# jac99/Egonn

Hardware: AMD Instinct MI355X
Metric: LiDAR scans/sec (descriptor extraction), 50k-pt clouds @ 0.1m voxel (higher is better)
Workload: dtype f32

## Files before the change

egonn_amd/_lib.py:

```python
from __future__ import annotations

import ctypes as C
import os
from typing import List, Optional, Sequence

import torch

_HERE = os.path.dirname(os.path.abspath(__file__))
LIB_PATH = os.path.join(_HERE, "lib", "libegonn_hip.so")

QUANT_CARTESIAN, QUANT_POLAR = 0, 1
FLAG_DISABLE_GLOBAL, FLAG_DISABLE_LOCAL, FLAG_IGNORE_KP_REGRESSOR, FLAG_BF16 = 1, 2, 4, 8
FLAG_POOL_SPOC, FLAG_POOL_MAC = 16, 32
MINKFPN_SPLIT_TOPDOWN = 1
MINKFPN_BLOCKS = {'BasicBlock': 0, 'ECABasicBlock': 1}
MINKFPN_POOLING = {None: 0, 'GeM': 1, 'MAC': 2, 'SPoC': 3}

_P = C.c_void_p
_SIGS = [
    ("egonn_ctx_create", C.c_int, [C.POINTER(_P), C.c_int, C.c_int]),
    ("egonn_ctx_destroy", None, [_P]),
    ("egonn_last_error", C.c_char_p, []),
    ("egonn_debug_set_naive_conv", C.c_int, [_P, C.c_int]),
    ("egonn_debug_set_ksplit", C.c_int, [_P, C.c_int, C.c_int, C.c_int, C.c_int, C.c_int]),
# ... 50 lines not shown
    ("egonn_minkfpn_finalize", C.c_int, [_P, C.c_int, C.POINTER(C.c_int), C.POINTER(C.c_int), C.c_int, C.c_int, C.c_int, C.c_int, _P]),
    ("egonn_minkfpn_out_level", C.c_int, [C.c_int, C.c_int, C.POINTER(C.c_int)]),
    ("egonn_minkfpn_forward", C.c_int, [_P, _P, C.c_int, _P, _P, _P]),
    ("egonn_topdown_step", C.c_int, [_P, C.c_int, _P, _P, _P, _P, C.c_int, C.c_int, _P, _P]),
    ("egonn_select_keypoints", C.c_int, [_P, _P, _P, _P, C.c_int, _P, _P, _P, _P, _P]),
    ("egonn_topk_rows", C.c_int, [_P, _P, C.c_int, C.c_int, _P, _P, _P]),
    ("egonn_triplet_loss_scratch_floats", C.c_int64, [C.c_int]),
    ("egonn_triplet_loss", C.c_int, [_P, C.c_int, C.c_int, _P, _P, C.c_float, _P, _P, _P, _P, _P]),
    ("egonn_nn_search", C.c_int, [_P, C.c_int64, _P, _P, C.c_int64, _P, _P, _P]),
    ("egonn_matrix_min", C.c_int, [_P, C.c_int64, C.c_int64, _P, _P, _P, _P, _P]),
    ("egonn_softmax_cross_entropy", C.c_int, [_P, C.c_int64, C.c_int64, _P, _P, _P, _P, _P]),
    ("egonn_local_loss_scratch_bytes", C.c_int64, [C.c_int, C.c_int64, C.c_int64, C.c_int]),
    ("egonn_local_loss", C.c_int, [C.c_int, C.c_int64, C.c_int64, C.c_int64, C.c_int64, C.c_int] + [_P] * 13 +
                                  [C.POINTER(C.c_float)] + [_P] * 9 + [C.c_int64, _P]),
    ("egonn_dense", C.c_int, [_P, C.c_int64, C.c_int, _P, C.c_int, _P, C.c_int, C.c_int, _P, _P]),
    ("egonn_dense_backward_weight", C.c_int, [_P, C.c_int, _P, C.c_int, C.c_int64, _P, _P, C.c_int64, _P]),
    ("egonn_conv_backward_weight", C.c_int, [_P, C.c_int, C.c_int, C.c_int, C.c_int, _P, C.c_int, _P, C.c_int, _P, _P,
                                             C.c_int64, _P]),
    ("egonn_col_stats", C.c_int, [C.c_int, _P, _P, _P, _P, C.c_int64, C.c_int, _P, _P, C.c_int64, _P]),
    ("egonn_bn_train_finalize", C.c_int, [_P, _P, C.c_double, C.c_int, _P, _P, C.c_float, C.c_float, _P, _P, _P, _P]),
    ("egonn_bn_backward_finalize", C.c_int, [_P, _P, C.c_double, C.c_int, _P, _P, _P, _P, _P]),
    ("egonn_affine_act", C.c_int, [_P, _P, _P, C.c_int64, C.c_int, C.c_int, _P, _P]),
    ("egonn_affine3", C.c_int, [_P, _P, _P, _P, _P, _P, C.c_int64, C.c_int, _P, _P]),
    ("egonn_relu_backward", C.c_int, [_P, _P, C.c_int64, C.c_int, _P, _P]),
    ("egonn_contrastive_loss_scratch_floats", C.c_int64, [C.c_int]),
    ("egonn_contrastive_loss", C.c_int, [_P, C.c_int, C.c_int, _P, _P, C.c_float, C.c_float, _P, _P, _P, _P, _P]),
    ("egonn_se_gate", C.c_int, [_P, _P, _P, _P, _P, C.c_int, C.c_int, C.c_int, _P, _P, _P]),
    ("egonn_se_gate_backward", C.c_int, [_P, _P, _P, _P, _P, _P, C.c_int, C.c_int, C.c_int, _P, _P, _P, _P, _P, _P]),
    ("egonn_eca_gate", C.c_int, [_P, _P, C.c_int, C.c_int, C.c_int, _P, _P]),
    ("egonn_eca_gate_backward", C.c_int, [_P, _P, _P, _P, C.c_int, C.c_int, C.c_int, _P, _P, _P]),
# ... 141 lines not shown
        raise ValueError(f"{name}: offsets must be a 1-D sequence of n_clouds + 1 entries, got shape {shape}")
    return shape[0] - 1


def concat_clouds(clouds, dev):
    ts = [torch.as_tensor(c) for c in clouds]
    for c in ts:
        check_cloud("cloud", c)
    off = [0]
    for c in ts:
        off.append(off[-1] + c.shape[0])
    pts = torch.cat([c.to(device=dev, dtype=torch.float32) for c in ts]) if ts else torch.zeros((0, 3), device=dev)
    return pts, torch.tensor(off, dtype=torch.int64, device=dev)


def debug_radix_sort(keys_in, vals_in, keys_out, vals_out, n: int, nbits: int, n_dev=None, seg_offsets=None, idx_bits: int = 0,
                     either_pair: bool = False, scratch_buf=None, scratch_bytes: Optional[int] = None) -> int:
    lib = load()
    B = 0 if seg_offsets is None else seg_offsets.numel() - 1
    need = lib.egonn_debug_radix_sort_scratch_bytes(int(n), B)
    if scratch_buf is None:
        scratch_buf = scratch(need, keys_in.device)
    pair = C.c_int32(-1)
    call(keys_in.device, lib.egonn_debug_radix_sort, keys_in.data_ptr(), vals_in.data_ptr(), keys_out.data_ptr(),
         vals_out.data_ptr(), int(n), int(nbits), _ptr(n_dev), _ptr(seg_offsets), B, int(idx_bits), int(bool(either_pair)),
         C.byref(pair), scratch_buf.data_ptr(), need if scratch_bytes is None else int(scratch_bytes))
    return pair.value


def require_gpu() -> torch.device:
# ... 561 lines not shown
```

egonn_amd/csrc/common.h:

```cpp
#pragma once
#include <hip/hip_runtime.h>
#include <atomic>
#include <stdint.h>
#include <stdio.h>
#include <string.h>
#include <string>
#include <vector>

#define EGONN_MAX_LEVELS 10
#define EGONN_NUM_LEVELS 8
#define EGONN_MAX_BATCH 4096

#define API extern "C" __attribute__((visibility("default")))

namespace egonn {

void set_error(const char* fmt, ...);
#define EGONN_OK 0
#define EGONN_ERR_INVALID 1
#define EGONN_ERR_HIP 2
#define EGONN_ERR_RANGE 3
#define EGONN_ERR_STATE 4
#define EGONN_ERR_CAPACITY 5
#define EGONN_ERR_FP16_RANGE 6
// ... 169 lines not shown
  hipEvent_t get();
};

struct Switches {
  bool debug_sync;
  bool no_presplit;
  bool no_fused_down;
  bool no_fused_lateral;
  bool no_gated_k2s2;
  bool no_fused_ghead;
  bool no_split_heads;
  bool no_tail_split;
  bool no_task_order;
  bool flat_sort, sort_pairs;
  bool no_search67;
  int split_max_level;
  int split_max_level_k8;
  int split_cfg;
  int rg_first_pass;
  const char* ksplit[5];
};
const Switches& switches();

struct KsRule {
  int8_t kparts[2][EGONN_NUM_LEVELS];
  int8_t kw[2][EGONN_NUM_LEVELS];
  int8_t col_parts[EGONN_NUM_LEVELS];
};

static constexpr int SCONV_RESIDENT_DEFAULT = 6;
// ... 76 lines not shown
```

egonn_amd/csrc/coords.hip:

```cpp
#include "common.h"

#include <algorithm>
#include <stdarg.h>

namespace egonn {

static thread_local char g_err[1024] = "";
void set_error(const char* fmt, ...) {
  va_list ap;
  va_start(ap, fmt);
  vsnprintf(g_err, sizeof(g_err), fmt, ap);
  va_end(ap);
}
const char* last_error() { return g_err; }

const Switches& switches() {
  static const Switches sw = [] {
    auto on = [](const char* name) { return getenv(name) != nullptr; };
    auto num = [](const char* name, int unset) { const char* e = getenv(name); return e ? atoi(e) : unset; };
    const char* ds = getenv("EGONN_DEBUG_SYNC");
    return Switches{.debug_sync = ds && ds[0] == '1', .no_presplit = on("EGONN_NO_PRESPLIT"), .no_fused_down = on("EGONN_NO_FUSED_DOWN"),
                    .no_fused_lateral = on("EGONN_NO_FUSED_LATERAL"), .no_gated_k2s2 = on("EGONN_NO_GATED_K2S2"),
                    .no_fused_ghead = on("EGONN_NO_FUSED_GHEAD"), .no_split_heads = on("EGONN_NO_SPLIT_HEADS"),
                    .no_tail_split = on("EGONN_NO_TAIL_SPLIT"), .no_task_order = on("EGONN_NO_TASK_ORDER"),
                    .flat_sort = on("EGONN_FLAT_SORT"), .sort_pairs = on("EGONN_SORT_PAIRS"), .no_search67 = on("EGONN_NO_SEARCH67"),
                    .split_max_level = num("EGONN_SPLIT_MAX_LEVEL", -1), .split_max_level_k8 = num("EGONN_SPLIT_MAX_LEVEL_K8", -1),
                    .split_cfg = num("EGONN_SPLIT_CFG", 0), .rg_first_pass = num("EGONN_RG_FIRST_PASS", 0),
                    .ksplit = {getenv("EGONN_KSPLIT"), getenv("EGONN_KSPLIT8"), getenv("EGONN_KSPLIT_KW"), getenv("EGONN_KSPLIT_KW8"),
                               getenv("EGONN_KSPLIT_PARTS")}};
  }();
  return sw;
}

hipEvent_t Profiler::get() {
  if (!pool.empty()) {
    hipEvent_t e = pool.back();
    pool.pop_back();
    return e;
  }
  hipEvent_t e = nullptr;
// ... 1037 lines not shown
```

egonn_amd/csrc/dense.hip:

```cpp
#include <algorithm>

#include "common.h"
#include "kernels.h"

namespace egonn {

typedef float f32x4 __attribute__((ext_vector_type(4)));

__device__ static inline float apply_act(float v, int act) {
  switch (act) {
    case ACT_RELU: return fmaxf(v, 0.f);
    case ACT_TANH: return tanhf(v);
    case ACT_SOFTPLUS: return v > 20.f ? v : log1pf(expf(v));
    case ACT_SIGMOID: return 1.f / (1.f + expf(-v));
    default: return v;
  }
}

__device__ static inline float bf2f(uint32_t h) { return __uint_as_float(h << 16); }
__device__ static inline uint32_t f2bf_rn(float a) {
  uint32_t u = __float_as_uint(a);
  u += 0x7FFFu + ((u >> 16) & 1u);
  return u >> 16;
}
// ... 338 lines not shown
          }
        }
        if (io & 2) {
          *reinterpret_cast<uint2*>(reinterpret_cast<uint16_t*>(out_v) + row * cout + c0) =
              make_uint2(f2bf_rn(v[0]) | (f2bf_rn(v[1]) << 16), f2bf_rn(v[2]) | (f2bf_rn(v[3]) << 16));
        } else {
          *reinterpret_cast<f32x4*>(reinterpret_cast<float*>(out_v) + row * cout + c0) = v;
        }
      }
    }
#pragma unroll
    for (int t = 0; t < KS; ++t) a[t] = an[t];
  }
}

__global__ void dense_any_kernel(const float* __restrict__ in, int64_t total, int cin, const float* __restrict__ W,
                                 int w_out_in, int cout, const float* __restrict__ bias, int act, float* __restrict__ out,
                                 const int32_t* __restrict__ n_dev) {
  const int64_t i = (int64_t)blockIdx.x * blockDim.x + threadIdx.x;
  if (n_dev) total = min((int64_t)*n_dev * cout, total);
  if (i >= total) return;
  const int64_t r = i / cout;
  const int co = (int)(i - r * cout);
  float s = bias ? bias[co] : 0.f;
  for (int ci = 0; ci < cin; ++ci) s = fmaf(in[r * cin + ci], w_out_in ? W[(int64_t)co * cin + ci] : W[(int64_t)ci * cout + co], s);
  out[i] = apply_act(s, act);
}

bool dense_gate_fusable(int64_t n, int cin, int cout) {
  const bool plan = cin == 32 || cin == 64 || cin == 96 || cin == 128 || cin == 192 || cin == 256;
  return plan && cout % 16 == 0 && n >= 8192 && (size_t)cin * cout * sizeof(float) <= 96 * 1024;
}

int dense_forward_ex(const void* in, int in_bf16, int64_t n, int cin, const float* W, int w_out_in, int cout,
                     const float* bias, const float* scale, const float* shift, int act, const void* residual, int res_bf16,
                     void* out, int out_bf16, hipStream_t stream, const int32_t* n_dev, const float* gate, const int32_t* boff,
                     int B) {
  if (n == 0) return EGONN_OK;
  EGONN_REQUIRE(!gate || (residual && boff && B >= 1 && dense_gate_fusable(n, cin, cout)), EGONN_ERR_INVALID,
                "dense: the fused gated residual needs the LDS-staged kernel (%lld rows, %d->%d)", (long long)n, cin, cout);
  const dim3 grid((unsigned)cdiv(n, 64), (unsigned)cdiv(cout, 64));
  const int io = (res_bf16 ? 1 : 0) | (out_bf16 ? 2 : 0);
  const size_t frag_bytes = (size_t)cin * cout * sizeof(float);
  const int ysplit = (int)cdiv((int64_t)frag_bytes, 96 * 1024);
  const int colblk = (int)(cdiv(cdiv(cout, ysplit), 16) * 16);
  if (cout % 16 == 0 && n >= (ysplit == 1 ? 8192 : 2048)) {
    const size_t blk_bytes = (size_t)cin * colblk * sizeof(float);
    const int ny = (int)cdiv(cout, colblk);
    const unsigned g1 = (unsigned)std::min<int64_t>(cdiv(cdiv(n, 16), 4), (blk_bytes > 72 * 1024 ? 256 : 512) / ny);
#define EGONN_DENSE_LDS_LAUNCH(WOI, CI, INB)                                                                           \
  {                                                                                                                   \
    static AttrOnce attr_done;                                                                                    \
    if (attr_done.need()) {                                                                                                 \
      HIP_CHECK(hipFuncSetAttribute(reinterpret_cast<const void*>(&dense_lds_kernel<WOI, CI, INB>),                   \
                                    hipFuncAttributeMaxDynamicSharedMemorySize, 160 * 1024));                         \
      attr_done.mark();                                                                                                \
    }                                                                                                                 \
// ... 981 lines not shown
  while (S < k) S <<= 1;
  const size_t lds = (size_t)(S + (k <= 512 ? k : 0)) * sizeof(unsigned long long);
  static AttrOnce attr_done;
  if (attr_done.need()) {
    HIP_CHECK(hipFuncSetAttribute(reinterpret_cast<const void*>(&select_topk_kernel), hipFuncAttributeMaxDynamicSharedMemorySize,
                                  128 * 1024));
    attr_done.mark(); 
  }
  hipLaunchKernelGGL(select_topk_kernel, dim3(B), dim3(TK_THREADS), lds, stream, sigma, boff_dev, k, S, kp, desc, dc, sel_rows,
                     sel_count, out_kp, out_desc);
  HIP_CHECK(hipGetLastError());
  return EGONN_OK;
}

}
```

egonn_amd/csrc/kernels.h:

```cpp
#pragma once
#include "common.h"

namespace egonn {

const char* last_error();

bool sconv_rg_supported(int cin, int cout);
int pack_rg_weights(const float* W, int K, int cin, int cout, int bf16, int flip, int transpose, void* out,
                    hipStream_t stream);
extern unsigned long long* g_sconv_trace;
struct PackedKernel {
  const void* rg32 = nullptr;
  const void* rg16 = nullptr;
  const void* split = nullptr;
};
struct ConvCall {
  int kind = 0, level = 0;
  const void* in = nullptr; void* out = nullptr;
  int cin = 0, cout = 0, bf16 = 0;
  const float *scale = nullptr, *shift = nullptr;
  int relu = 0;
  float* psum = nullptr;
  const PackedKernel* packed = nullptr;
  const float* W = nullptr; float* scratch = nullptr; size_t scratch_floats = 0;
// ... 44 lines not shown
int sconv_naive(const float* in, const int32_t* nbr, const float* W, const float* scale, const float* shift, int relu,
                float* out, int64_t n_out, int K, int cin, int cout, hipStream_t stream);
int conv0_lut_init(Ctx* ctx);
int conv0_k5_forward(Ctx* ctx, const float* feat, const float* W, int cout, const float* scale,
                     const float* shift, int relu, void* out, int out_bf16, hipStream_t stream, const void* wpk = nullptr);
int conv0_pack_unit(const float* W, void* wpk, hipStream_t stream);

enum Act { ACT_NONE = 0, ACT_RELU = 1, ACT_TANH = 2, ACT_SOFTPLUS = 3, ACT_SIGMOID = 4 };
int dense_forward(const float* in, int64_t n, int cin, const float* W, int w_out_in, int cout, const float* bias,
                  const float* scale, const float* shift, int act, const float* residual, float* out,
                  hipStream_t stream);
bool dense_gate_fusable(int64_t n, int cin, int cout);
int dense_forward_ex(const void* in, int in_bf16, int64_t n, int cin, const float* W, int w_out_in, int cout,
                     const float* bias, const float* scale, const float* shift, int act, const void* residual, int res_bf16,
                     void* out, int out_bf16, hipStream_t stream, const int32_t* n_dev = nullptr, const float* gate = nullptr,
                     const int32_t* boff = nullptr, int B = 0);
int bn_fold(const float* w, const float* b, const float* rm, const float* rv, float eps, int c, float* scale,
            float* shift, hipStream_t stream);
int gather_rows(const float* in, const int32_t* perm, int64_t n, int c, float* out, hipStream_t stream,
                const int32_t* n_dev = nullptr);
static constexpr int SEG_CHUNKS = 32;
int segment_partial_sums(const float* in, const int32_t* boff, int B, int c, int pow_mode, const float* p,
                         float* partial, hipStream_t stream);
int eca_apply(const float* x, const float* res, const float* partial, const int32_t* boff, int B, int64_t n, int c,
              const float* wconv, int ksize, float* out, hipStream_t stream);
int eca_gate_groups(const float* psum, const RowGroups& rg, const int32_t* boff, int B, int c, const float* wconv, int ksize,
                    float* gate, hipStream_t stream);
int eca_apply_gate(const void* x, const void* res, const float* gate, const int32_t* boff, int B, int64_t n, int c,
                   void* out, int bf16, hipStream_t stream);
int convert_bf16_to_f32(const void* in, int64_t n, float* out, hipStream_t stream);
int gem_finish(const float* partial, const int32_t* boff, int B, int c, const float* p, float* out,
// ... 34 lines not shown
```

egonn_amd/csrc/model.h:

```cpp
#pragma once
#include <map>
#include <string>
#include <vector>

#include "../../include/egonn_hip.h"
#include "common.h"
#include "kernels.h"

struct egonn_ctx : public egonn::Ctx {
  hipStream_t plan_stream = nullptr;

  void* level_feat[EGONN_NUM_LEVELS] = {};
  int level_ch[EGONN_NUM_LEVELS] = {};
  int level_bf16 = 0;
  bool from_points = false;
};

#define REQUIRE_PLAN(c)                                                                               \
  EGONN_REQUIRE((c) && (c)->plan.valid, EGONN_ERR_STATE, "no coordinate plan (call egonn_voxelize / " \
                                                         "egonn_coords_set first)")
#define REQUIRE_LEVEL(c, level)                                                                              \
  REQUIRE_PLAN(c);                                                                                           \
  HIP_CHECK(hipSetDevice((c)->device));                                                                      \
  EGONN_REQUIRE((level) >= 0 && (level) < EGONN_NUM_LEVELS, EGONN_ERR_INVALID, "level %d out of range", (level))
// ... 34 lines not shown
  float* folded = nullptr;
  size_t folded_cap = 0;
  const float* conv0 = nullptr;
  egonn::BnRef bn[8];
  const float* convs[8] = {};
  egonn::BlockRef blk[8];
  const float *g1x1[8] = {}, *gt[8] = {}, *l1x1[8] = {}, *lt[8] = {};
  const float* gem_p = nullptr;
  egonn::MlpRef gdec, ldec, kp, sg;
  float* packed = nullptr;
  size_t packed_cap = 0;
  void* conv0_unit = nullptr;
  void* lh_pack = nullptr;
  const float** lh_ptrs = nullptr;
  egonn::PackedKernel pk_convs[8], pk_c1[8], pk_c2[8], pk_gt[8], pk_lt[8];
  egonn::MinkFpnModel* fpn = nullptr;
};

namespace egonn {

int get_tensor(egonn_model* m, const std::string& key, std::initializer_list<int64_t> want, const float** out);
int get_bn(egonn_model* m, const std::string& prefix, int c, BnRef* bn, float** cursor);
int fold(const BnRef& bn, hipStream_t st);
int conv_layer(egonn_ctx* c, hipStream_t st, const ConvCall& cc, const char* what);
ConvCall conv_call(int kind, int level, const void* in, const PackedKernel& pk, int cin, int cout, int bf16, const BnRef* bn, int relu,
                   void* out);

bool topdown_split_supported(int C, int Cl);
int topdown_split_forward(Ctx* ctx, int level_out, const float* x_coarse, const void* sp_tconv, const float* x_lateral,
                          const void* sp_lateral, int C, int Cl, float* out, hipStream_t stream);
// ... 3 lines not shown
```

egonn_amd/csrc/model.hip:

```cpp
#include "model.h"

using namespace egonn;

namespace {

const int PLANES[7] = {32, 64, 64, 128, 128, 128, 128};
const int GLOBAL_CH = 128, GLOBAL_DIM = 256, LOCAL_CH = 64, LOCAL_DIM = 128;

}

API const char* egonn_last_error(void) { return last_error(); }

API int egonn_debug_set_naive_conv(egonn_ctx* c, int on) {
  EGONN_REQUIRE(c, EGONN_ERR_INVALID, "debug_set_naive_conv: null context");
  if (on >= 1000) { c->conv_variant = on; return EGONN_OK; }
  c->conv_variant = (on == 1) ? 3 : (on == 2 ? 1 : (on == 4 ? 2 : (on == 8 ? 4 : (on == 16 ? 5 : (on == 32 ? 6 : (on == 128 ? 9 : 0))))));
  return EGONN_OK;
}

API int egonn_debug_set_ksplit(egonn_ctx* c, int map_class, int level, int kparts, int kw, int col_parts) {
  EGONN_REQUIRE(c && (map_class == 0 || map_class == 1) && level >= 0 && level < EGONN_NUM_LEVELS, EGONN_ERR_INVALID,
                "debug_set_ksplit: bad argument");
  EGONN_REQUIRE(kparts <= 27 && kw <= 4 && col_parts <= 4, EGONN_ERR_INVALID, "debug_set_ksplit: kparts <= 27, kw <= 4, col_parts <= 4");
  if (kparts >= 0) c->ks_rule.kparts[map_class][level] = (int8_t)std::max(kparts, 1);
// ... 623 lines not shown
  EGONN_TRY(get_tensor(m, "local_head.tconv.4.kernel", {8, LOCAL_CH, LOCAL_CH}, &m->lt[4]));
  m->gem_p = nullptr;
  if (m->t.count("global_pooling.pooling.p")) EGONN_TRY(get_tensor(m, "global_pooling.pooling.p", {1}, &m->gem_p));
  EGONN_TRY(get_mlp(m, "global_descriptor_decoder", GLOBAL_CH, GLOBAL_DIM + (GLOBAL_CH - GLOBAL_DIM) / 2, GLOBAL_DIM, &m->gdec));
  EGONN_TRY(get_mlp(m, "local_descriptor_decoder", LOCAL_CH, LOCAL_DIM + (LOCAL_CH - LOCAL_DIM) / 2, LOCAL_DIM, &m->ldec));
  EGONN_TRY(get_mlp(m, "local_keypoint_regressor", LOCAL_CH, LOCAL_CH / 2, 3, &m->kp));
  EGONN_TRY(get_mlp(m, "local_sigma_regressor", LOCAL_CH, LOCAL_CH / 2, 1, &m->sg));

  {
    size_t need_p = 0;
    for (int i = 1; i <= 7; ++i) {
      const BlockRef& b = m->blk[i];
      need_p += (size_t)8 * b.cin * b.cin + (size_t)27 * b.cin * b.cout + (size_t)27 * b.cout * b.cout;
    }
    need_p += (size_t)2 * 8 * GLOBAL_CH * GLOBAL_CH + (size_t)8 * LOCAL_CH * LOCAL_CH;
    if (m->packed_cap < need_p) {
      if (m->packed) HIP_CHECK(hipFree(m->packed));
      HIP_CHECK(hipMalloc(reinterpret_cast<void**>(&m->packed), (3 * need_p + 512) * sizeof(float)));
      m->packed_cap = need_p;
    }
    float* pc = m->packed;
    uint16_t* qc = reinterpret_cast<uint16_t*>(m->packed + need_p);
    uint16_t* sc = reinterpret_cast<uint16_t*>(m->packed + need_p + need_p / 2 + 16);
    auto pack2 = [&](const float* w, int K, int ci, int co, PackedKernel* dst) -> int {
      EGONN_TRY(pack_rg_weights(w, K, ci, co, 0, 0, 0, pc, st));
      EGONN_TRY(pack_rg_weights(w, K, ci, co, 1, 0, 0, qc, st));
      *dst = PackedKernel{pc, qc, nullptr};
      if (sconv_split_supported(ci, co)) {
        EGONN_TRY(pack_split_weights(w, K, ci, co, 0, 0, sc, st));
        dst->split = sc;
        sc += split_weights_bytes(K, ci, co) / 2;
      }
      pc += (size_t)K * ci * co;
      qc += (size_t)K * ci * co;
      return EGONN_OK;
    };
    for (int i = 1; i <= 7; ++i) {
      const BlockRef& b = m->blk[i];
      EGONN_TRY(pack2(m->convs[i], 8, b.cin, b.cin, &m->pk_convs[i]));
      EGONN_TRY(pack2(b.conv1, 27, b.cin, b.cout, &m->pk_c1[i]));
      EGONN_TRY(pack2(b.conv2, 27, b.cout, b.cout, &m->pk_c2[i]));
    }
    EGONN_TRY(pack2(m->gt[6], 8, GLOBAL_CH, GLOBAL_CH, &m->pk_gt[6]));
    EGONN_TRY(pack2(m->gt[7], 8, GLOBAL_CH, GLOBAL_CH, &m->pk_gt[7]));
    EGONN_TRY(pack2(m->lt[4], 8, LOCAL_CH, LOCAL_CH, &m->pk_lt[4]));
  }
  if (!m->conv0_unit) HIP_CHECK(hipMalloc(&m->conv0_unit, 2 * 4 * 3 * 64 * 16));
  EGONN_TRY(conv0_pack_unit(m->conv0, m->conv0_unit, st));
  if (m->ldec.cin == 64 && m->ldec.mid == 96 && m->ldec.cout == 128 && m->kp.mid == 32 && m->sg.mid == 32 && m->kp.cin == 64 &&
      m->sg.cin == 64) {
    if (!m->lh_pack) HIP_CHECK(hipMalloc(&m->lh_pack, local_heads_pack_bytes()));
    if (!m->lh_ptrs) HIP_CHECK(hipMalloc(reinterpret_cast<void**>(&m->lh_ptrs), 6 * sizeof(float*)));
    const float* hp[6] = {m->ldec.w0, m->ldec.w1, m->kp.w0, m->kp.w1, m->sg.w0, m->sg.w1};
    HIP_CHECK(hipMemcpyAsync(m->lh_ptrs, hp, sizeof(hp), hipMemcpyHostToDevice, st));
    HIP_CHECK(hipStreamSynchronize(st));
    EGONN_TRY(local_heads_pack(m->lh_ptrs, m->lh_pack, st));
  }
  EGONN_TRY(fold(m->bn[0], st));
  for (int i = 1; i <= 7; ++i) {
    EGONN_TRY(fold(m->bn[i], st));
// ... 99 lines not shown
  }
  FALLOC(x0, n0 * 32);
  {
    ProfScope ps(c, st, "conv0_k5_kernel/L0", PK_CONV0, 0, 125, 1, 32, (int)es);
    EGONN_TRY(conv0_k5_forward(c, f0, m->conv0, 32, m->bn[0].scale, m->bn[0].shift, 1, x0, bf16, st, m->conv0_unit));
  }
  DBG_SYNC("conv0");
  const void* x[8] = {x0};
  c->level_feat[0] = x0;
  c->level_ch[0] = 32;
  c->level_bf16 = bf16;
  auto local_head = [&](hipStream_t st) -> int {
    const int64_t n3 = P.cap[3], n4 = P.cap[4];
    FALLOC(l4, n4 * LOCAL_CH);
    EGONN_TRY(dense_forward_ex(x[4], bf16, n4, 128, m->l1x1[4], 0, LOCAL_CH, nullptr, nullptr, nullptr, ACT_NONE, nullptr, 0, l4,
                               bf16, st, cnt + 4));
    FALLOC(u3, n3 * LOCAL_CH);
    EGONN_TRY(conv_layer(c, st, conv_call(2, 3, l4, m->pk_lt[4], LOCAL_CH, LOCAL_CH, bf16, nullptr, 0, u3), "tconv"));
    EGONN_REQUIRE(m->ldec.cin == 64 && m->ldec.mid == 96 && m->ldec.cout == 128 && m->kp.mid == 32 && m->sg.mid == 32,
                  EGONN_ERR_STATE, "local heads: unexpected layer sizes");
    const float* hw[12] = {m->ldec.w0, m->ldec.b0, m->ldec.w1, m->ldec.b1, m->kp.w0, m->kp.b0, m->kp.w1, m->kp.b1,
                           m->sg.w0, m->sg.b0, m->sg.w1, m->sg.b1};
    const void* lh_pack = (!switches().no_split_heads && sconv_split_arithmetic(c)) ? m->lh_pack : nullptr;
    if (!switches().no_fused_lateral && LOCAL_CH == 64) {
      EGONN_TRY(local_heads_forward(reinterpret_cast<const float*>(x[3]), n3, cnt + 3, hw, P.lv[3].keys, 3, P.coord_bits, quant_mode,
                                    step, (flags & EGONN_FLAG_IGNORE_KP_REGRESSOR) ? 1 : 0, out_desc, out_kp, out_sigma, st,
                                    m->l1x1[3], reinterpret_cast<const float*>(u3), bf16, lh_pack, c->dev_fp16_flag));
      return EGONN_OK;
    }
    WALLOC(l3, n3 * LOCAL_CH);
    EGONN_TRY(dense_forward_ex(x[3], bf16, n3, 64, m->l1x1[3], 0, LOCAL_CH, nullptr, nullptr, nullptr, ACT_NONE, u3, bf16, l3, 0, st, cnt + 3));
    EGONN_TRY(local_heads_forward(l3, n3, cnt + 3, hw, P.lv[3].keys, 3, P.coord_bits, quant_mode, step,
                                  (flags & EGONN_FLAG_IGNORE_KP_REGRESSOR) ? 1 : 0, out_desc, out_kp, out_sigma, st, nullptr, nullptr, 0,
                                  lh_pack, c->dev_fp16_flag));
    return EGONN_OK;
  };
  const float *gated_t2 = nullptr, *gated_res = nullptr, *gated_gate = nullptr;
  for (int i = 1; i <= 7; ++i) {
    const BlockRef& b = m->blk[i];
    const Level& L = P.lv[i];
    const int64_t n = P.cap[i];
    FALLOC(y, n * b.cin);
    {
      ConvCall cc = conv_call(1, i, x[i - 1], m->pk_convs[i], b.cin, b.cin, bf16, &m->bn[i], 1, y);
      if (gated_t2 && i == 2) {
        cc.in = gated_t2;
// ... 25 lines not shown
    DBG_SYNC("L%d eca gate", i);
    const void* res = y;
    if (i == 1 && !switches().no_gated_k2s2 && !c->keep_level_features && !bf16 && !b.down && c->conv_variant == 0 && b.cout == 32 &&
        m->blk[2].cin == 32 && sconv_route(c, 1, 2, 32, 32, 0) == ROUTE_SPLIT) {
      gated_t2 = reinterpret_cast<const float*>(t2);
      gated_res = reinterpret_cast<const float*>(y);
      gated_gate = gate;
      x[i] = nullptr;
      c->level_feat[i] = nullptr;
      c->level_ch[i] = b.cout;
      continue;
    }
    FALLOC(xo, n * b.cout);
    if (b.down && !switches().no_fused_down && dense_gate_fusable(n, b.cin, b.cout)) {
      EGONN_TRY(dense_forward_ex(y, bf16, n, b.cin, b.down, 0, b.cout, nullptr, b.dn.scale, b.dn.shift, ACT_NONE, t2, bf16, xo,
                                 bf16, st, cnt + i, gate, L.boff, B));
    } else {
      if (b.down) {
        FALLOC(rd, n * b.cout);
        EGONN_TRY(dense_forward_ex(y, bf16, n, b.cin, b.down, 0, b.cout, nullptr, b.dn.scale, b.dn.shift, ACT_NONE, nullptr, 0, rd,
                                   bf16, st, cnt + i));
        res = rd;
      }
      EGONN_TRY(eca_apply_gate(t2, res, gate, L.boff, B, n, b.cout, xo, bf16, st));
    }
    DBG_SYNC("L%d eca apply", i);
    x[i] = xo;
    c->level_feat[i] = xo;
    c->level_ch[i] = b.cout;
  }
  if (do_local) EGONN_TRY(local_head(st));
  DBG_SYNC("local head");

  void* g5_fused = nullptr;
  if (do_global && !switches().no_fused_ghead && !bf16 && c->conv_variant == 0 && P.cap[5] < 8192 && P.cap[6] < 8192 && P.cap[7] < 8192) {
    WALLOC(l7, P.cap[7] * GLOBAL_CH);
// ... 146 lines not shown
```

include/egonn_hip.h:

```cpp
#ifndef EGONN_HIP_H
#define EGONN_HIP_H

#include <stdint.h>

#ifdef __cplusplus
extern "C" {
#endif

typedef struct egonn_ctx egonn_ctx;
typedef struct egonn_model egonn_model;

enum { EGONN_QUANT_CARTESIAN = 0, EGONN_QUANT_POLAR = 1 };
enum { EGONN_STATUS_OK = 0, EGONN_STATUS_INVALID = 1, EGONN_STATUS_HIP = 2, EGONN_STATUS_RANGE = 3, EGONN_STATUS_STATE = 4,
       EGONN_STATUS_CAPACITY = 5,
       EGONN_STATUS_FP16_RANGE = 6 };
enum { EGONN_FLAG_DISABLE_GLOBAL = 1, EGONN_FLAG_DISABLE_LOCAL = 2, EGONN_FLAG_IGNORE_KP_REGRESSOR = 4,
       EGONN_FLAG_BF16 = 8,
       EGONN_FLAG_POOL_SPOC = 16, EGONN_FLAG_POOL_MAC = 32 };

int egonn_ctx_create(egonn_ctx** ctx, int device, int coord_bits);
void egonn_ctx_destroy(egonn_ctx* ctx);
const char* egonn_last_error(void);
int egonn_debug_set_naive_conv(egonn_ctx* ctx, int on);
int egonn_debug_set_ksplit(egonn_ctx* ctx, int map_class, int level, int kparts, int kw, int col_parts);
// ... 120 lines not shown
       EGONN_LL_CHAMFER_WEIGHTED = 4, EGONN_LL_MEAN_SIGMA = 5, EGONN_LL_LOSS_CHAMFER = 6, EGONN_LL_LOSS_P2P = 7,
       EGONN_LL_KEYPOINT_LOSS = 8, EGONN_LL_CORRESPONDENCE_LOSS = 9, EGONN_LL_MATCHING_KEYPOINTS = 10,
       EGONN_LL_MATCHING_DESCRIPTORS = 11, EGONN_LL_POS_SIMILARITY = 12, EGONN_LL_NEG_SIMILARITY = 13  };
int64_t egonn_local_loss_scratch_bytes(int pairs, int64_t n_kp1, int64_t n_kp2, int dim);
int egonn_local_loss(int pairs, int64_t n_cloud1, int64_t n_cloud2, int64_t n_kp1, int64_t n_kp2, int dim,
                     const float* clouds1, const int32_t* cloud_off1, const float* clouds2, const int32_t* cloud_off2,
                     const float* kp1, const float* sigma1, const float* desc1, const int32_t* kp_off1,
                     const float* kp2, const float* sigma2, const float* desc2, const int32_t* kp_off2,
                     const float* transforms, const float* params, float* out_pair, float* out_batch,
                     float* g_kp1, float* g_sigma1, float* g_desc1, float* g_kp2, float* g_sigma2, float* g_desc2,
                     void* scratch, int64_t scratch_bytes, void* stream);

enum { EGONN_ACT_NONE = 0, EGONN_ACT_RELU = 1, EGONN_ACT_TANH = 2, EGONN_ACT_SOFTPLUS = 3, EGONN_ACT_SIGMOID = 4 };
int egonn_dense(const float* x, int64_t n, int cin, const float* weight, int weight_out_in, const float* bias, int cout,
                int act, float* out, void* stream);
int egonn_dense_backward_weight(const float* a, int ca, const float* b, int cb, int64_t n, float* out, float* scratch,
                                int64_t scratch_floats, void* stream);
int egonn_conv_backward_weight(egonn_ctx* ctx, int level_in, int level_out, int kernel_size, int transposed,
                               const float* in, int cin, const float* grad_out, int cout, float* grad_kernel,
                               float* scratch, int64_t scratch_floats, void* stream);
int egonn_col_stats(int mode, const float* a, const float* b, const float* mask, const float* mean, int64_t n, int c,
                    double* out, float* scratch, int64_t scratch_floats, void* stream);
int egonn_bn_train_finalize(const double* sums, const float* shift_point, double count, int c, const float* weight,
                            const float* bias, float eps, float momentum, float* running_mean, float* running_var,
                            float* out_mean_invstd_scale_shift, void* stream);
int egonn_bn_backward_finalize(const double* local_sums, const double* global_sums, double count, int c, const float* weight,
                               const float* mean, const float* invstd, float* out_abc_dgamma_dbeta, void* stream);
int egonn_affine_act(const float* x, const float* scale, const float* shift, int64_t n, int c, int relu, float* out,
                     void* stream);
int egonn_affine3(const float* g, const float* mask, const float* x, const float* A, const float* B, const float* C,
// ... 157 lines not shown
```

Measured before the change: 22450.

## Add streaming MFMA dense kernel with prepacked weight fragments for 1x1 layers

Adds a dense (1x1 conv) kernel specialised by template on channel count. Each wave handles 16 rows, loads the whole weight matrix into LDS as MFMA-ready fragments, and fuses bias, scale/shift, activation, residual and gated residual into the epilogue. The weights for the downsample and lateral 1x1 layers are packed into fragment order once at model finalize, so the kernel skips the per-launch reordering. This aims to cut per-row overhead and register tiling waste for large point counts. It adds template instantiations, more LDS per block, and a new default path for n>=8192 that can be turned off with EGONN_NO_DENSE_STREAM.

```diff
diff --git a/egonn_amd/_lib.py b/egonn_amd/_lib.py
--- a/egonn_amd/_lib.py
+++ b/egonn_amd/_lib.py
@@ -4,6 +4,7 @@
 import os
 from typing import List, Optional, Sequence
 
+import numpy as np
 import torch
 
 _HERE = os.path.dirname(os.path.abspath(__file__))
@@ -88,6 +89,10 @@
     ("egonn_local_loss", C.c_int, [C.c_int, C.c_int64, C.c_int64, C.c_int64, C.c_int64, C.c_int] + [_P] * 13 +
                                   [C.POINTER(C.c_float)] + [_P] * 9 + [C.c_int64, _P]),
     ("egonn_dense", C.c_int, [_P, C.c_int64, C.c_int, _P, C.c_int, _P, C.c_int, C.c_int, _P, _P]),
+    ("egonn_dense_pack_fragments", C.c_int, [_P, C.c_int, C.c_int, C.c_int, _P, _P]),
+    ("egonn_dense_pack_fragments_host", C.c_int, [_P, C.c_int, C.c_int, C.c_int, _P]),
+    ("egonn_debug_dense", C.c_int, [_P, C.c_int, C.c_int64, _P, C.c_int, C.c_int, _P, C.c_int, _P, _P, _P, _P, C.c_int, _P, C.c_int,
+                                    _P, _P, C.c_int, _P, C.c_int, C.c_int, _P]),
     ("egonn_dense_backward_weight", C.c_int, [_P, C.c_int, _P, C.c_int, C.c_int64, _P, _P, C.c_int64, _P]),
     ("egonn_conv_backward_weight", C.c_int, [_P, C.c_int, C.c_int, C.c_int, C.c_int, _P, C.c_int, _P, C.c_int, _P, _P,
                                              C.c_int64, _P]),
@@ -259,6 +264,33 @@
     return pts, torch.tensor(off, dtype=torch.int64, device=dev)
 
 
+def dense_pack_fragments(weight, out_in: bool):
+    lib = load()
+    co, ci = (weight.shape if out_in else weight.shape[::-1])
+    if isinstance(weight, np.ndarray):
+        w = np.ascontiguousarray(weight, dtype=np.float32)
+        out = np.empty(ci * co, dtype=np.float32)
+        check(lib.egonn_dense_pack_fragments_host(w.ctypes.data, int(bool(out_in)), int(ci), int(co), out.ctypes.data))
+        return out
+    w = weight.contiguous()
+    out = torch.empty(ci * co, dtype=torch.float32, device=w.device)
+    call(w.device, lib.egonn_dense_pack_fragments, w.data_ptr(), int(bool(out_in)), int(ci), int(co), out.data_ptr())
+    return out
+
+
+def debug_dense(x, weight, out_in: bool, out, form: int, n_dev=None, packed=None, bias=None, scale=None, shift=None, act: int = 0,
+                residual=None, gate=None, boff=None):
+    lib = load()
+    cap, cin = x.shape
+    cout = out.shape[1]
+    B = 0 if boff is None else boff.numel() - 1
+    bf = lambda t: int(t is not None and t.dtype == torch.bfloat16)
+    call(x.device, lib.egonn_debug_dense, x.data_ptr(), bf(x), int(cap), _ptr(n_dev), int(cin), int(cout), weight.data_ptr(),
+         int(bool(out_in)), _ptr(packed), _ptr(bias), _ptr(scale), _ptr(shift), int(act), _ptr(residual), bf(residual), _ptr(gate),
+         _ptr(boff), B, out.data_ptr(), bf(out), int(form))
+    return out
+
+
 def debug_radix_sort(keys_in, vals_in, keys_out, vals_out, n: int, nbits: int, n_dev=None, seg_offsets=None, idx_bits: int = 0,
                      either_pair: bool = False, scratch_buf=None, scratch_bytes: Optional[int] = None) -> int:
     lib = load()
diff --git a/egonn_amd/csrc/common.h b/egonn_amd/csrc/common.h
--- a/egonn_amd/csrc/common.h
+++ b/egonn_amd/csrc/common.h
@@ -207,6 +207,7 @@
   bool no_task_order;
   bool flat_sort, sort_pairs;
   bool no_search67;
+  bool no_dense_stream;
   int split_max_level;
   int split_max_level_k8;
   int split_cfg;
diff --git a/egonn_amd/csrc/coords.hip b/egonn_amd/csrc/coords.hip
--- a/egonn_amd/csrc/coords.hip
+++ b/egonn_amd/csrc/coords.hip
@@ -24,6 +24,7 @@
                     .no_fused_ghead = on("EGONN_NO_FUSED_GHEAD"), .no_split_heads = on("EGONN_NO_SPLIT_HEADS"),
                     .no_tail_split = on("EGONN_NO_TAIL_SPLIT"), .no_task_order = on("EGONN_NO_TASK_ORDER"),
                     .flat_sort = on("EGONN_FLAT_SORT"), .sort_pairs = on("EGONN_SORT_PAIRS"), .no_search67 = on("EGONN_NO_SEARCH67"),
+                    .no_dense_stream = on("EGONN_NO_DENSE_STREAM"),
                     .split_max_level = num("EGONN_SPLIT_MAX_LEVEL", -1), .split_max_level_k8 = num("EGONN_SPLIT_MAX_LEVEL_K8", -1),
                     .split_cfg = num("EGONN_SPLIT_CFG", 0), .rg_first_pass = num("EGONN_RG_FIRST_PASS", 0),
                     .ksplit = {getenv("EGONN_KSPLIT"), getenv("EGONN_KSPLIT8"), getenv("EGONN_KSPLIT_KW"), getenv("EGONN_KSPLIT_KW8"),
diff --git a/egonn_amd/csrc/dense.hip b/egonn_amd/csrc/dense.hip
--- a/egonn_amd/csrc/dense.hip
+++ b/egonn_amd/csrc/dense.hip
@@ -376,6 +376,163 @@
   }
 }
 
+__host__ __device__ static inline int64_t dense_frag_src(int64_t j, int w_out_in, int cin, int cout) {
+  const int u = (int)(j & 3), ln = (int)((j >> 2) & 63), ft = (int)(j >> 8), ks = cin / 16;
+  const int nt = ft / ks, t = ft - nt * ks;
+  const int ci = 16 * t + 4 * (ln >> 4) + u, col = 16 * nt + (ln & 15);
+  return w_out_in ? (int64_t)col * cin + ci : (int64_t)ci * cout + col;
+}
+__global__ void dense_pack_kernel(const float* __restrict__ W, int w_out_in, int cin, int cout, float* __restrict__ out) {
+  const int64_t j = (int64_t)blockIdx.x * blockDim.x + threadIdx.x;
+  if (j < (int64_t)cin * cout) out[j] = W[dense_frag_src(j, w_out_in, cin, cout)];
+}
+int dense_pack_frags(const float* W, int w_out_in, int cin, int cout, float* out, hipStream_t stream) {
+  EGONN_REQUIRE(W && out && cin >= 16 && cin % 16 == 0 && cout >= 16 && cout % 16 == 0, EGONN_ERR_INVALID,
+                "dense pack: %d->%d (multiples of 16 expected)", cin, cout);
+  hipLaunchKernelGGL(dense_pack_kernel, dim3((unsigned)cdiv((int64_t)cin * cout, 256)), dim3(256), 0, stream, W, w_out_in ? 1 : 0, cin,
+                     cout, out);
+  HIP_CHECK(hipGetLastError());
+  return EGONN_OK;
+}
+
+template <int CIN, int COUT, bool IN_BF16, bool ACT_ANY>
+__global__ __launch_bounds__(256, 4) void dense_stream_kernel(const void* __restrict__ in_v, int64_t n, const float* __restrict__ W,
+                                                           int w_out_in, const float* __restrict__ wfrag,
+                                                           const float* __restrict__ bias, const float* __restrict__ scale,
+                                                           const float* __restrict__ shift, int act,
+                                                           const void* __restrict__ residual_v, void* __restrict__ out_v, int io,
+                                                           const int32_t* __restrict__ n_dev, const float* __restrict__ gate,
+                                                           const int32_t* __restrict__ boff, int B) {
+  extern __shared__ __attribute__((aligned(16))) f32x4 ds_frags[];
+  constexpr int KS = CIN / 16, NT = COUT / 16, NFRAG = NT * KS * 64, PER = NFRAG / 256;
+  static_assert(NFRAG % 256 == 0, "whole fragments per thread");
+  float* const s_vec = reinterpret_cast<float*>(ds_frags + NFRAG);
+  int32_t* const s_boff = reinterpret_cast<int32_t*>(s_vec + 3 * COUT);
+  if (n_dev) n = min((int64_t)*n_dev, n);
+  if (!gate) B = 0;
+  const int tid = threadIdx.x, lane = tid & 63, wave = tid >> 6;
+  const int l15 = lane & 15, g4 = lane >> 4;
+  f32x4 st[PER];
+  {
+    const f32x4* src = reinterpret_cast<const f32x4*>(wfrag ? wfrag : W);
+#pragma unroll
+    for (int u = 0; u < PER; ++u) st[u] = src[tid + u * 256];
+  }
+  const int vi = min(tid, COUT - 1);
+  float vb = (bias ? bias : W)[vi], vs = (scale ? scale : W)[vi], vh = (scale ? shift : W)[vi];
+  const int32_t vo = (gate ? boff : reinterpret_cast<const int32_t*>(W))[gate ? min(tid, B) : 0];
+  const int64_t row = ((int64_t)blockIdx.x * 4 + wave) * 16 + l15;
+  const bool ok = row < n;
+  const int64_t rowc = min(row, max(n, (int64_t)1) - 1);
+  f32x4 a[KS], r[NT];
+#pragma unroll
+  for (int t = 0; t < KS; ++t) {
+    if constexpr (IN_BF16) {
+      const uint2 h = *reinterpret_cast<const uint2*>(reinterpret_cast<const uint16_t*>(in_v) + rowc * CIN + 16 * t + 4 * g4);
+      a[t] = (f32x4){__uint_as_float(h.x), __uint_as_float(h.y), 0.f, 0.f};
+    } else {
+      a[t] = *reinterpret_cast<const f32x4*>(reinterpret_cast<const float*>(in_v) + rowc * CIN + 16 * t + 4 * g4);
+    }
+  }
+  {
+    const void* rp = residual_v ? residual_v : static_cast<const void*>(W);
+    const int64_t r0 = (residual_v ? rowc * COUT : 0) + 4 * g4;
+    if (io & 1) {
+#pragma unroll
+      for (int nt = 0; nt < NT; ++nt) {
+        const uint2 h = *reinterpret_cast<const uint2*>(reinterpret_cast<const uint16_t*>(rp) + r0 + 16 * nt);
+        r[nt] = (f32x4){__uint_as_float(h.x), __uint_as_float(h.y), 0.f, 0.f};
+      }
+    } else {
+#pragma unroll
+      for (int nt = 0; nt < NT; ++nt) r[nt] = *reinterpret_cast<const f32x4*>(reinterpret_cast<const float*>(rp) + r0 + 16 * nt);
+    }
+  }
+#pragma unroll
+  for (int u = 0; u < PER; ++u) ds_frags[tid + u * 256] = st[u];
+  if (!wfrag) {
+#pragma unroll 1
+    for (int i = tid; i < NFRAG; i += 256) {
+      f32x4 v;
+#pragma unroll
+      for (int k = 0; k < 4; ++k) v[k] = W[dense_frag_src((int64_t)i * 4 + k, w_out_in, CIN, COUT)];
+      ds_frags[i] = v;
+    }
+  }
+  if (tid < COUT) {
+    s_vec[tid] = bias ? vb : 0.f;
+    s_vec[COUT + tid] = scale ? vs : 1.f;
+    s_vec[2 * COUT + tid] = scale ? vh : 0.f;
+  }
+  if (tid <= B) s_boff[tid] = vo;
+  for (int i = tid + 256; i <= B; i += 256) s_boff[i] = boff[i];
+  __syncthreads();
+  if (((int64_t)blockIdx.x * 4 + wave) * 16 >= n) return;
+  f32x4 gq[NT];
+  {
+    int lo = 0, hi = gate ? B : 0;
+    while (hi - lo > 1) {
+      const int mid = (lo + hi) >> 1;
+      if (s_boff[mid] <= (int32_t)row) lo = mid; else hi = mid;
+    }
+    const float* gp = (gate ? gate : W) + ((gate && ok) ? (int64_t)lo * COUT : 0) + 4 * g4;
+#pragma unroll
+    for (int nt = 0; nt < NT; ++nt) gq[nt] = *reinterpret_cast<const f32x4*>(gp + 16 * nt);
+  }
+  __builtin_amdgcn_sched_barrier(0);
+  if constexpr (IN_BF16) {
+#pragma unroll
+    for (int t = 0; t < KS; ++t) {
+      const uint32_t hx = __float_as_uint(a[t][0]), hy = __float_as_uint(a[t][1]);
+      a[t] = (f32x4){bf2f(hx & 0xFFFFu), bf2f(hx >> 16), bf2f(hy & 0xFFFFu), bf2f(hy >> 16)};
+    }
+  }
+#pragma unroll
+  for (int nt = 0; nt < NT; ++nt) {
+    f32x4 acc = {0.f, 0.f, 0.f, 0.f};
+    const f32x4* fr = ds_frags + nt * KS * 64 + lane;
+#pragma unroll
+    for (int t = 0; t < KS; ++t) {
+      const f32x4 wf = fr[t * 64];
+#pragma unroll
+      for (int u = 0; u < 4; ++u) acc = __builtin_amdgcn_mfma_f32_16x16x4f32(wf[u], a[t][u], acc, 0, 0, 0);
+    }
+    if (ok) {
+      const int c0 = 16 * nt + 4 * g4;
+      f32x4 v = acc + *reinterpret_cast<const f32x4*>(s_vec + c0);
+      v = v * *reinterpret_cast<const f32x4*>(s_vec + COUT + c0) + *reinterpret_cast<const f32x4*>(s_vec + 2 * COUT + c0);
+#pragma unroll
+      for (int u = 0; u < 4; ++u) v[u] = ACT_ANY ? apply_act(v[u], act) : (act == ACT_RELU ? fmaxf(v[u], 0.f) : v[u]);
+      if (residual_v) {
+        f32x4 rr = r[nt];
+        if (io & 1) {
+          const uint32_t hx = __float_as_uint(rr[0]), hy = __float_as_uint(rr[1]);
+          rr = (f32x4){bf2f(hx & 0xFFFFu), bf2f(hx >> 16), bf2f(hy & 0xFFFFu), bf2f(hy >> 16)};
+        }
+        if (gate) {
+#pragma unroll
+          for (int u = 0; u < 4; ++u) {
+            const float d = (io & 2) ? bf2f(f2bf_rn(v[u])) : v[u];
+            v[u] = fmaxf(rr[u] * gq[nt][u] + d, 0.f);
+          }
+        } else {
+          v += rr;
+        }
+      }
+      if (io & 2) {
+        *reinterpret_cast<uint2*>(reinterpret_cast<uint16_t*>(out_v) + row * COUT + c0) =
+            make_uint2(f2bf_rn(v[0]) | (f2bf_rn(v[1]) << 16), f2bf_rn(v[2]) | (f2bf_rn(v[3]) << 16));
+      } else {
+        *reinterpret_cast<f32x4*>(reinterpret_cast<float*>(out_v) + row * COUT + c0) = v;
+      }
+    }
+    __builtin_amdgcn_sched_barrier(0);
+  }
+}
+static bool dense_stream_shape(int64_t n, int cin, int cout) {
+  return n >= 8192 && (cin == 32 || cin == 64 || cin == 128) && (cout == 64 || cout == 128) && (size_t)cin * cout * sizeof(float) <= 32 * 1024;
+}
+
 __global__ void dense_any_kernel(const float* __restrict__ in, int64_t total, int cin, const float* __restrict__ W,
                                  int w_out_in, int cout, const float* __restrict__ bias, int act, float* __restrict__ out,
                                  const int32_t* __restrict__ n_dev) {
@@ -397,12 +554,39 @@
 int dense_forward_ex(const void* in, int in_bf16, int64_t n, int cin, const float* W, int w_out_in, int cout,
                      const float* bias, const float* scale, const float* shift, int act, const void* residual, int res_bf16,
                      void* out, int out_bf16, hipStream_t stream, const int32_t* n_dev, const float* gate, const int32_t* boff,
-                     int B) {
+                     int B, const float* wfrag, int form) {
   if (n == 0) return EGONN_OK;
   EGONN_REQUIRE(!gate || (residual && boff && B >= 1 && dense_gate_fusable(n, cin, cout)), EGONN_ERR_INVALID,
                 "dense: the fused gated residual needs the LDS-staged kernel (%lld rows, %d->%d)", (long long)n, cin, cout);
+  EGONN_REQUIRE(form != 1 || dense_stream_shape(n, cin, cout), EGONN_ERR_INVALID, "dense: no streaming form for %lld rows, %d->%d",
+                (long long)n, cin, cout);
   const dim3 grid((unsigned)cdiv(n, 64), (unsigned)cdiv(cout, 64));
   const int io = (res_bf16 ? 1 : 0) | (out_bf16 ? 2 : 0);
+  if (form == 1 || (form < 0 && !switches().no_dense_stream && dense_stream_shape(n, cin, cout))) {
+    const unsigned g1 = (unsigned)cdiv(cdiv(n, 16), 4);
+    const size_t lds = (size_t)cin * cout * sizeof(float) + 3 * (size_t)cout * sizeof(float) + ((size_t)(gate ? B : 0) + 1) * sizeof(int32_t);
+    const bool act_any = act != ACT_NONE && act != ACT_RELU;
+#define EGONN_DENSE_STREAM_LAUNCH(CI, CO, INB, ANY)                                                                                  \
+  if ((in_bf16 != 0) == INB && act_any == ANY)                                                                                       \
+    hipLaunchKernelGGL((dense_stream_kernel<CI, CO, INB, ANY>), dim3(g1), dim3(256), lds, stream, in, n, W, w_out_in, wfrag, bias,  \
+                       scale, shift, act, residual, out, io, n_dev, gate, boff, B);
+#define EGONN_DENSE_STREAM_CASE(CI, CO)                                                                                              \
+  if (cin == CI && cout == CO) {                                                                                                     \
+    EGONN_DENSE_STREAM_LAUNCH(CI, CO, true, true)                                                                                    \
+    EGONN_DENSE_STREAM_LAUNCH(CI, CO, true, false)                                                                                   \
+    EGONN_DENSE_STREAM_LAUNCH(CI, CO, false, true)                                                                                   \
+    EGONN_DENSE_STREAM_LAUNCH(CI, CO, false, false)                                                                                  \
+    HIP_CHECK(hipGetLastError());                                                                                                    \
+    return EGONN_OK;                                                                                                                 \
+  }
+    EGONN_DENSE_STREAM_CASE(32, 64)
+    EGONN_DENSE_STREAM_CASE(32, 128)
+    EGONN_DENSE_STREAM_CASE(64, 64)
+    EGONN_DENSE_STREAM_CASE(64, 128)
+    EGONN_DENSE_STREAM_CASE(128, 64)
+#undef EGONN_DENSE_STREAM_CASE
+#undef EGONN_DENSE_STREAM_LAUNCH
+  }
   const size_t frag_bytes = (size_t)cin * cout * sizeof(float);
   const int ysplit = (int)cdiv((int64_t)frag_bytes, 96 * 1024);
   const int colblk = (int)(cdiv(cdiv(cout, ysplit), 16) * 16);
@@ -1414,3 +1598,25 @@
 }
 
 }
+
+using namespace egonn;
+
+API int egonn_dense_pack_fragments(const float* weight, int weight_out_in, int cin, int cout, float* packed, void* stream) {
+  return dense_pack_frags(weight, weight_out_in, cin, cout, packed, (hipStream_t)stream);
+}
+API int egonn_dense_pack_fragments_host(const float* weight, int weight_out_in, int cin, int cout, float* packed) {
+  EGONN_REQUIRE(weight && packed && cin >= 16 && cin % 16 == 0 && cout >= 16 && cout % 16 == 0, EGONN_ERR_INVALID,
+                "dense pack: %d->%d (multiples of 16 expected)", cin, cout);
+  for (int64_t j = 0; j < (int64_t)cin * cout; ++j) packed[j] = weight[dense_frag_src(j, weight_out_in ? 1 : 0, cin, cout)];
+  return EGONN_OK;
+}
+API int egonn_debug_dense(const void* in, int in_bf16, int64_t rows_capacity, const int32_t* n_dev, int cin, int cout, const float* weight,
+                          int weight_out_in, const float* packed, const float* bias, const float* scale, const float* shift, int act,
+                          const void* residual, int res_bf16, const float* gate, const int32_t* boff, int B, void* out, int out_bf16,
+                          int form, void* stream) {
+  EGONN_REQUIRE(in && weight && out && rows_capacity >= 0 && cin >= 1 && cout >= 1 && act >= 0 && act <= 4 && (form == 0 || form == 1) &&
+                    (!scale == !shift) && (form == 1 || !packed),
+                EGONN_ERR_INVALID, "debug_dense: bad arguments");
+  return dense_forward_ex(in, in_bf16 ? 1 : 0, rows_capacity, cin, weight, weight_out_in ? 1 : 0, cout, bias, scale, shift, act, residual,
+                          res_bf16 ? 1 : 0, out, out_bf16 ? 1 : 0, (hipStream_t)stream, n_dev, gate, boff, B, packed, form);
+}
diff --git a/egonn_amd/csrc/kernels.h b/egonn_amd/csrc/kernels.h
--- a/egonn_amd/csrc/kernels.h
+++ b/egonn_amd/csrc/kernels.h
@@ -82,7 +82,9 @@
 int dense_forward_ex(const void* in, int in_bf16, int64_t n, int cin, const float* W, int w_out_in, int cout,
                      const float* bias, const float* scale, const float* shift, int act, const void* residual, int res_bf16,
                      void* out, int out_bf16, hipStream_t stream, const int32_t* n_dev = nullptr, const float* gate = nullptr,
-                     const int32_t* boff = nullptr, int B = 0);
+                     const int32_t* boff = nullptr, int B = 0,
+                     const float* wfrag = nullptr, int form = -1);
+int dense_pack_frags(const float* W, int w_out_in, int cin, int cout, float* out, hipStream_t stream);
 int bn_fold(const float* w, const float* b, const float* rm, const float* rv, float eps, int c, float* scale,
             float* shift, hipStream_t stream);
 int gather_rows(const float* in, const int32_t* perm, int64_t n, int c, float* out, hipStream_t stream,
diff --git a/egonn_amd/csrc/model.h b/egonn_amd/csrc/model.h
--- a/egonn_amd/csrc/model.h
+++ b/egonn_amd/csrc/model.h
@@ -72,6 +72,7 @@
   void* lh_pack = nullptr;
   const float** lh_ptrs = nullptr;
   egonn::PackedKernel pk_convs[8], pk_c1[8], pk_c2[8], pk_gt[8], pk_lt[8];
+  const float *pk_down[8] = {}, *pk_l1x1[8] = {};
   egonn::MinkFpnModel* fpn = nullptr;
 };
 
diff --git a/egonn_amd/csrc/model.hip b/egonn_amd/csrc/model.hip
--- a/egonn_amd/csrc/model.hip
+++ b/egonn_amd/csrc/model.hip
@@ -661,6 +661,9 @@
       need_p += (size_t)8 * b.cin * b.cin + (size_t)27 * b.cin * b.cout + (size_t)27 * b.cout * b.cout;
     }
     need_p += (size_t)2 * 8 * GLOBAL_CH * GLOBAL_CH + (size_t)8 * LOCAL_CH * LOCAL_CH;
+    for (int i = 1; i <= 7; ++i)
+      if (m->blk[i].down) need_p += (size_t)m->blk[i].cin * m->blk[i].cout;
+    for (int l : {3, 4}) need_p += (size_t)PLANES[l - 1] * LOCAL_CH;
     if (m->packed_cap < need_p) {
       if (m->packed) HIP_CHECK(hipFree(m->packed));
       HIP_CHECK(hipMalloc(reinterpret_cast<void**>(&m->packed), (3 * need_p + 512) * sizeof(float)));
@@ -691,6 +694,19 @@
     EGONN_TRY(pack2(m->gt[6], 8, GLOBAL_CH, GLOBAL_CH, &m->pk_gt[6]));
     EGONN_TRY(pack2(m->gt[7], 8, GLOBAL_CH, GLOBAL_CH, &m->pk_gt[7]));
     EGONN_TRY(pack2(m->lt[4], 8, LOCAL_CH, LOCAL_CH, &m->pk_lt[4]));
+    auto pack1 = [&](const float* w, int ci, int co, const float** dst) -> int {
+      *dst = nullptr;
+      if (ci % 16 || co % 16) return EGONN_OK;
+      EGONN_TRY(dense_pack_frags(w, 0, ci, co, pc, st));
+      *dst = pc;
+      pc += (size_t)ci * co;
+      return EGONN_OK;
+    };
+    for (int i = 1; i <= 7; ++i) {
+      m->pk_down[i] = nullptr;
+      if (m->blk[i].down) EGONN_TRY(pack1(m->blk[i].down, m->blk[i].cin, m->blk[i].cout, &m->pk_down[i]));
+    }
+    for (int l : {3, 4}) EGONN_TRY(pack1(m->l1x1[l], PLANES[l - 1], LOCAL_CH, &m->pk_l1x1[l]));
   }
   if (!m->conv0_unit) HIP_CHECK(hipMalloc(&m->conv0_unit, 2 * 4 * 3 * 64 * 16));
   EGONN_TRY(conv0_pack_unit(m->conv0, m->conv0_unit, st));
@@ -820,7 +836,7 @@
     const int64_t n3 = P.cap[3], n4 = P.cap[4];
     FALLOC(l4, n4 * LOCAL_CH);
     EGONN_TRY(dense_forward_ex(x[4], bf16, n4, 128, m->l1x1[4], 0, LOCAL_CH, nullptr, nullptr, nullptr, ACT_NONE, nullptr, 0, l4,
-                               bf16, st, cnt + 4));
+                               bf16, st, cnt + 4, nullptr, nullptr, 0, m->pk_l1x1[4]));
     FALLOC(u3, n3 * LOCAL_CH);
     EGONN_TRY(conv_layer(c, st, conv_call(2, 3, l4, m->pk_lt[4], LOCAL_CH, LOCAL_CH, bf16, nullptr, 0, u3), "tconv"));
     EGONN_REQUIRE(m->ldec.cin == 64 && m->ldec.mid == 96 && m->ldec.cout == 128 && m->kp.mid == 32 && m->sg.mid == 32,
@@ -835,7 +851,8 @@
       return EGONN_OK;
     }
     WALLOC(l3, n3 * LOCAL_CH);
-    EGONN_TRY(dense_forward_ex(x[3], bf16, n3, 64, m->l1x1[3], 0, LOCAL_CH, nullptr, nullptr, nullptr, ACT_NONE, u3, bf16, l3, 0, st, cnt + 3));
+    EGONN_TRY(dense_forward_ex(x[3], bf16, n3, 64, m->l1x1[3], 0, LOCAL_CH, nullptr, nullptr, nullptr, ACT_NONE, u3, bf16, l3, 0, st, cnt + 3,
+                               nullptr, nullptr, 0, m->pk_l1x1[3]));
     EGONN_TRY(local_heads_forward(l3, n3, cnt + 3, hw, P.lv[3].keys, 3, P.coord_bits, quant_mode, step,
                                   (flags & EGONN_FLAG_IGNORE_KP_REGRESSOR) ? 1 : 0, out_desc, out_kp, out_sigma, st, nullptr, nullptr, 0,
                                   lh_pack, c->dev_fp16_flag));
@@ -891,12 +908,12 @@
     FALLOC(xo, n * b.cout);
     if (b.down && !switches().no_fused_down && dense_gate_fusable(n, b.cin, b.cout)) {
       EGONN_TRY(dense_forward_ex(y, bf16, n, b.cin, b.down, 0, b.cout, nullptr, b.dn.scale, b.dn.shift, ACT_NONE, t2, bf16, xo,
-                                 bf16, st, cnt + i, gate, L.boff, B));
+                                 bf16, st, cnt + i, gate, L.boff, B, m->pk_down[i]));
     } else {
       if (b.down) {
         FALLOC(rd, n * b.cout);
         EGONN_TRY(dense_forward_ex(y, bf16, n, b.cin, b.down, 0, b.cout, nullptr, b.dn.scale, b.dn.shift, ACT_NONE, nullptr, 0, rd,
-                                   bf16, st, cnt + i));
+                                   bf16, st, cnt + i, nullptr, nullptr, 0, m->pk_down[i]));
         res = rd;
       }
       EGONN_TRY(eca_apply_gate(t2, res, gate, L.boff, B, n, b.cout, xo, bf16, st));
diff --git a/include/egonn_hip.h b/include/egonn_hip.h
--- a/include/egonn_hip.h
+++ b/include/egonn_hip.h
@@ -158,6 +158,12 @@
 enum { EGONN_ACT_NONE = 0, EGONN_ACT_RELU = 1, EGONN_ACT_TANH = 2, EGONN_ACT_SOFTPLUS = 3, EGONN_ACT_SIGMOID = 4 };
 int egonn_dense(const float* x, int64_t n, int cin, const float* weight, int weight_out_in, const float* bias, int cout,
                 int act, float* out, void* stream);
+int egonn_dense_pack_fragments(const float* weight, int weight_out_in, int cin, int cout, float* packed, void* stream);
+int egonn_dense_pack_fragments_host(const float* weight, int weight_out_in, int cin, int cout, float* packed);
+int egonn_debug_dense(const void* in, int in_bf16, int64_t rows_capacity, const int32_t* n_dev, int cin, int cout, const float* weight,
+                      int weight_out_in, const float* packed, const float* bias, const float* scale, const float* shift, int act,
+                      const void* residual, int res_bf16, const float* gate, const int32_t* boff, int B, void* out, int out_bf16,
+                      int form, void* stream);
 int egonn_dense_backward_weight(const float* a, int ca, const float* b, int cb, int64_t n, float* out, float* scratch,
                                 int64_t scratch_floats, void* stream);
 int egonn_conv_backward_weight(egonn_ctx* ctx, int level_in, int level_out, int kernel_size, int transposed,
```

Measured after the change: 22760, median of 6. 1.01x the previous value.
